# chrischoy/DeepGlobalRegistration

Hardware: AMD Instinct MI355X
Metric: pair registrations/sec (FCGF x2 + 1-NN + 6-D inlier net + gate + weighted Procrustes + SE(3) refinement) (higher is better)
Workload: dtype f32 results via 2 x f16 split operands (3 f16 MFMA products per MAC, f32 accumulate); k = 1 convs, kNN re-evaluation and registration in exact f32, SVD in f64

## Files before the change

deepglobalregistration_amd/csrc/conv_wide.hip:

```cpp
#include <stdlib.h>

#include <type_traits>

#include "dgr_internal.h"
#include "split.h"

struct ConvWideArgs {
  const unsigned char *planes;
  const float *row_scale;
  float *y;
  const uint4 *wb;
  int64_t piece_stride;
  const int32_t *pair_in, *tile_ptr;
  int cout, K;
  float w_unscale;
  unsigned long long *clk;
};

#define DGR_LDS_PTR(off) ((__attribute__((address_space(3))) void *)(lds + (off)))
#define DGR_GLOBAL_PTR(p) ((const __attribute__((address_space(1))) void *)(p))

template <int N>
__device__ __forceinline__ void dgr_wait_vmcnt() {
  static_assert(N >= 0 && N < 64, "vmcnt is a 6-bit counter");
  asm volatile("s_waitcnt vmcnt(%0)" ::"n"(N) : "memory");
}
__device__ __forceinline__ void dgr_phase_barrier() {
  asm volatile("s_waitcnt lgkmcnt(0)\n\ts_barrier" ::: "memory");
}

__host__ __device__ constexpr int dgr_wide_passes(int h, int npass, int nsp) {
  return h < nsp ? npass / nsp + (h < npass % nsp ? 1 : 0) : 0;
}
__host__ __device__ constexpr int dgr_wide_pass_base(int h, int npass, int nsp) {
  int b = 0;
  for (int i = 0; i < h; ++i) b += dgr_wide_passes(i, npass, nsp);
  return b;
}

template <int CP, int NB, int WM>
__global__ void __launch_bounds__(512, 1) sparse_conv_wide_f16x2(ConvWideArgs a, const int4 *__restrict__ tdesc) {
  constexpr int NCW = 4;
  constexpr int NP = 2, MB = 2 / WM, WN = NCW / WM, PW = 4, TM = 64, CK = 64, SK = CK / 16;
  static_assert(WM == 1 || WM == 2, "row split of the compute waves");
  static_assert(TM == DGR_TILE_M && CP % CK == 0, "shape");
  constexpr int PPT = CP / CK, S = CP / 16, NBLK = NB * WN, COUT = 32 * NBLK;
  static_assert(PPT == 1 || PPT == 2 || PPT == 4, "a round of NSET phases is a whole number of tiles");
  constexpr int ROWB = 4 * CP;
  constexpr int NBUF = 3;
  constexpr int NSET = 4;
  constexpr int LEAD = NSET + 2;
  constexpr int BUFB = TM * 256;
  constexpr int RING = 16;
  constexpr int AH_I = 8, AH_S = 4;
  static_assert(RING >= 2 * AH_I && AH_I > LEAD && AH_S >= 3 && AH_S < AH_I, "ring distances");
  constexpr int WD = NB >= 2 ? 2 : 4;
  static_assert(SK % WD == 0, "the weight ring turns a whole number of times per phase (static register indexing)");
  constexpr int LDS_ST = COUT + 4;
  constexpr int NSTG = PPT == 1 ? 2 : 1;
  constexpr int HB = PPT / 2;
  constexpr int RPH = TM / PPT;
  constexpr int PD = 2;
  constexpr int PTH = 64 * (PW - PD);
  constexpr int CPR = COUT / 4;
  constexpr int RPP = PTH / CPR;
  constexpr int NPS = RPH / RPP;
  static_assert(RPH % RPP == 0, "store passes");
  constexpr int OFF_STAGE = NBUF * BUFB;
  constexpr int OFF_IDX = OFF_STAGE + NSTG * TM * LDS_ST * 4;
  constexpr int OFF_SC = OFF_IDX + RING * TM * 4;
  constexpr int LDS_BYTES = OFF_SC + RING * TM * 4;
  static_assert(LDS_BYTES <= 160 * 1024, "LDS budget");
  __shared__ __attribute__((aligned(16))) unsigned char lds[LDS_BYTES];

  const int tid = threadIdx.x;
  const int lane = tid & 63;
  const int wave = __builtin_amdgcn_readfirstlane(tid >> 6);
  if (a.clk && tid == 0) atomicMin(a.clk, (unsigned long long)wall_clock64());
  const int T = a.tile_ptr[a.K];
  const int per = (T + 7) >> 3;
  const int xcd = blockIdx.x & 7;
  const int t_end = min(T, (xcd + 1) * per);
  const int nj = gridDim.x >> 3;
  const int t_first = xcd * per + (blockIdx.x >> 3);
  if (t_first >= t_end) return;
  const int n_my = (t_end - t_first + nj - 1) / nj;
  const int n_loop = n_my + 2;
  auto desc = [&](int i) -> int4 { return tdesc[t_first + min(max(i, 0), n_my - 1) * nj]; };
  auto stage_of = [&](int t) -> float * {
    return reinterpret_cast<float *>(lds + OFF_STAGE) + (NSTG == 2 ? (t & 1) : 0) * TM * LDS_ST;
  };

  if (wave >= NCW) {
    const int pw = wave - NCW;
    if (pw < PD) {
      constexpr int RW = TM / PD, NI = RW / 4;
      f32x4 G[NSET][NI];
      const unsigned char *rb[NI];
      auto row_bases = [&](int i) {
        const int *idx = reinterpret_cast<const int *>(lds + OFF_IDX + (i & (RING - 1)) * TM * 4);
#pragma unroll
        for (int jj = 0; jj < NI; ++jj) {
          const int r = RW * pw + 4 * jj + (lane >> 4);
          rb[jj] = a.planes + (int64_t)idx[r] * ROWB + 16 * ((lane & 15) ^ (r & 15));
        }
      };
      auto request = [&](int p, f32x4 *Gs) {
        if (p % PPT == 0) row_bases(p / PPT);
#pragma unroll
        for (int jj = 0; jj < NI; ++jj) Gs[jj] = *reinterpret_cast<const f32x4 *>(rb[jj] + (p % PPT) * 256);
      };
      auto land = [&](int p, const f32x4 *Gs) {
        unsigned char *dst = lds + (p % NBUF) * BUFB + (NI * pw) * 1024 + lane * 16;
#pragma unroll
        for (int jj = 0; jj < NI; ++jj) *reinterpret_cast<f32x4 *>(dst + jj * 1024) = Gs[jj];
      };
      int *ring_i = reinterpret_cast<int *>(lds + OFF_IDX);
      float *ring_s = reinterpret_cast<float *>(lds + OFF_SC);
      auto load_idx = [&](int i) -> int {
        const int4 d = desc(i);
        return a.pair_in[d.y + min(lane, d.z - 1)];
      };
#pragma unroll
      for (int i = 0; i < AH_I - 1; ++i) ring_i[i * TM + lane] = load_idx(i);
#pragma unroll
      for (int i = 0; i < AH_S - 1; ++i) ring_s[i * TM + lane] = a.row_scale[ring_i[i * TM + lane]];
      int idx_reg = load_idx(AH_I - 1);
      float sc_reg = a.row_scale[ring_i[(AH_S - 1) * TM + lane]];
      auto rings = [&](int t) {
        ring_i[((t + AH_I - 1) & (RING - 1)) * TM + lane] = idx_reg;
        ring_s[((t + AH_S - 1) & (RING - 1)) * TM + lane] = sc_reg;
        idx_reg = load_idx(t + AH_I);
        sc_reg = a.row_scale[ring_i[((t + AH_S) & (RING - 1)) * TM + lane]];
      };
      dgr_phase_barrier();
#pragma unroll
      for (int j = 0; j < NSET; ++j) request(j, G[j]);
      land(0, G[0]); request(NSET, G[0]);
      land(1, G[1]); request(NSET + 1, G[1]);
      dgr_phase_barrier();
      auto phase = [&](int q, f32x4 *Gs) {
        if (q % PPT == 0) rings(q / PPT);
        land(q + 2, Gs);
        request(q + LEAD, Gs);
        dgr_phase_barrier();
      };
      for (int q = 0; q < n_loop * PPT; q += NSET) {
        phase(q, G[2]);
        if (q + 1 < n_loop * PPT) phase(q + 1, G[3]);
        if (q + 2 < n_loop * PPT) phase(q + 2, G[0]);
        if (q + 3 < n_loop * PPT) phase(q + 3, G[1]);
      }
      return;
    }
    const int ptid = tid - 64 * (NCW + PD);
    auto store_rows = [&](int u, int r0) {
      if (u < 0 || u >= n_my) return;
      const int4 d = desc(u);
      const float *sc = reinterpret_cast<const float *>(lds + OFF_SC + (u & (RING - 1)) * TM * 4);
      const float *st = stage_of(u);
      const int c4 = (ptid % CPR) * 4;
      f32x4 v[NPS];
#pragma unroll
      for (int i = 0; i < NPS; ++i) {
        const int r = r0 + i * RPP + ptid / CPR;
        v[i] = *reinterpret_cast<const f32x4 *>(st + r * LDS_ST + c4);
        v[i] *= dgr_inv_pow2(sc[r]) * a.w_unscale;
      }
#pragma unroll
      for (int i = 0; i < NPS; ++i) {
        const int r = r0 + i * RPP + ptid / CPR;
        if (r < d.z) __builtin_nontemporal_store(v[i], reinterpret_cast<f32x4 *>(a.y + (int64_t)(d.y + r) * COUT + c4));
      }
    };
    dgr_phase_barrier();
    dgr_phase_barrier();
    auto sphase = [&](int t, auto hc) {
      constexpr int h = decltype(hc)::value;
      if constexpr (h == 0) store_rows(t - 2, (PPT - 1) * RPH);
      else store_rows(t - 1, (h - 1) * RPH);
      dgr_phase_barrier();
    };
    for (int t = 0; t < n_loop; ++t) {
      sphase(t, std::integral_constant<int, 0>());
      if constexpr (PPT > 1) sphase(t, std::integral_constant<int, 1>());
      if constexpr (PPT > 2) {
        sphase(t, std::integral_constant<int, 2>());
        sphase(t, std::integral_constant<int, 3>());
      }
    }
    if (a.clk && lane == 0) {
      dgr_wait_vmcnt<0>();
      atomicMax(a.clk + 1, (unsigned long long)wall_clock64());
    }
    return;
  }

  const int wn = wave % WN, wm = wave / WN;
  int4 dc = desc(0), dn = desc(1);
  uint4 w[WD][NB][NP];
  auto wload = [&](int k, int s, uint4 (*ws)[NP]) {
    const uint4 *p = a.wb + ((int64_t)(k * S + s) * NBLK + wn * NB) * 64 + lane;
#pragma unroll
    for (int j = 0; j < NB; ++j)
#pragma unroll
      for (int pc = 0; pc < NP; ++pc) ws[j][pc] = p[(int64_t)pc * a.piece_stride + j * 64];
  };
#pragma unroll
  for (int g = 0; g < WD - 1; ++g) wload(dc.x, g % S, w[g]);
  dgr_phase_barrier();
  dgr_phase_barrier();
  uint4 op[2][MB][NP];
  const int lofs0 = (32 * MB * wm + (lane & 31)) * 256 + 16 * ((lane >> 5) ^ (lane & 15));
  auto oload = [&](int b, int s, uint4 (*o)[NP]) {
    const unsigned char *p = lds + b * BUFB + (lofs0 ^ (32 * s));
    const unsigned char *pm = lds + b * BUFB + (lofs0 ^ (32 * s) ^ 128);
#pragma unroll
    for (int i = 0; i < MB; ++i) {
      o[i][0] = *reinterpret_cast<const uint4 *>(p + i * 32 * 256);
      o[i][1] = *reinterpret_cast<const uint4 *>(pm + i * 32 * 256);
    }
  };
  oload(0, 0, op[0]);
  int buf = 0;
  constexpr int NPC = (4 * NB + SK - 1) / SK;
  auto stage_pieces = [&](float *st, const f32x16 (&ac)[MB][NB], int i, int s) {
    float *dst = st + (32 * (MB * wm + i) + (lane & 31)) * LDS_ST;
#pragma unroll
    for (int u = 0; u < NPC; ++u) {
      const int wq = s * NPC + u, j = wq / 4, g = wq % 4;
      if (wq < 4 * NB) {
        const int col = 32 * (wn * NB + j) + 8 * g + 4 * (lane >> 5);
        *reinterpret_cast<f32x4 *>(dst + col) = f32x4{ac[i][j][4 * g], ac[i][j][4 * g + 1], ac[i][j][4 * g + 2], ac[i][j][4 * g + 3]};
      }
    }
  };
  auto ctile = [&](int t, f32x16 (&ac)[MB][NB], const f32x16 (&ad)[MB][NB]) {
    const bool stage_prev = t >= 1 && t <= n_my;
    float *st = stage_of(t - 1);
#pragma unroll
    for (int h = 0; h < PPT; ++h) {
      if (h == 0) {
#pragma unroll
        for (int i = 0; i < MB; ++i)
#pragma unroll
          for (int j = 0; j < NB; ++j)
#pragma unroll
            for (int e = 0; e < 16; ++e) ac[i][j][e] = 0.f;
      }
      const int nbuf = buf == NBUF - 1 ? 0 : buf + 1;
      const int s0 = h * SK;
#pragma unroll
      for (int s = 0; s < SK; ++s) {
        {
          const int sg = s0 + s + WD - 1;
          wload(sg < S ? dc.x : dn.x, sg < S ? sg : sg - S, w[(s + WD - 1) % WD]);
        }
        if (s + 1 < SK) oload(buf, s + 1, op[(s + 1) & 1]);
        else oload(nbuf, 0, op[0]);
        __builtin_amdgcn_sched_barrier(0);
        uint4 (*wc)[NP] = w[s % WD];
        uint4 (*oc)[NP] = op[s & 1];
#define DGR_WIDE_TERM(WP, OP)                                                                                         \
  _Pragma("unroll") for (int i = 0; i < MB; ++i) _Pragma("unroll") for (int j = 0; j < NB; ++j)                       \
      ac[i][j] = __builtin_amdgcn_mfma_f32_32x32x16_f16(__builtin_bit_cast(f16x8, wc[j][WP]),                          \
                                                        __builtin_bit_cast(f16x8, oc[i][OP]), ac[i][j], 0, 0, 0);
        DGR_WIDE_TERM(1, 0)
        DGR_WIDE_TERM(0, 1)
        DGR_WIDE_TERM(0, 0)
#undef DGR_WIDE_TERM
        if (stage_prev) {
          if (h == 0) stage_pieces(st, ad, 0, s);
          if constexpr (MB > 1) {
            if (h == HB) stage_pieces(st, ad, 1, s);
          }
        }
      }
      if (h == PPT - 1) {
        dc = dn;
        dn = desc(t + 2);
      }
      buf = nbuf;
      dgr_phase_barrier();
    }
  };
  f32x16 accA[MB][NB], accB[MB][NB];
  for (int t = 0; t < n_loop; t += 2) {
    ctile(t, accA, accB);
    if (t + 1 < n_loop) ctile(t + 1, accB, accA);
  }
  if (a.clk && lane == 0) atomicMax(a.clk + 1, (unsigned long long)wall_clock64());
}

template <int CP, int NB, int WM>
static int launch_wide(const ConvWideArgs &ka, const int4 *tile_desc, int64_t tile_bound, int num_cus, hipStream_t stream) {
  int64_t grid = num_cus;
  if (tile_bound < grid) grid = tile_bound;
  grid = (grid + 7) / 8 * 8;
  if (grid < 8) grid = 8;
  sparse_conv_wide_f16x2<CP, NB, WM><<<(int)grid, 512, 0, stream>>>(ka, tile_desc);
  DGR_LAUNCH_CHECK();
  return DGR_OK;
}

bool dgr_conv_wide_supported(int cin_pad, int cin, int cout) {
  if (cin != cin_pad) return false;
  return (cout == 64 && cin == 64) || (cout == 128 && (cin == 64 || cin == 128 || cin == 256)) ||
         (cout == 256 && (cin == 128 || cin == 256));
}

int dgr_conv_wide_launch(const DgrConvLaunch &a, const DgrSplitRows &in, const void *wb, int64_t piece_stride,
                         float w_unscale, int num_cus, hipStream_t stream, const char **kernel_name) {
  DGR_REQUIRE(a.pair_in && wb && in.planes && in.scale && dgr_conv_wide_supported(a.cin_pad, a.cin, a.cout),
              "wide conv: unsupported layer (Cin %d, Cout %d) or no split input rows", a.cin, a.cout);
  DGR_REQUIRE(in.channels == a.cin, "wide conv: the split rows have %d channels, the layer %d", in.channels, a.cin);
  DGR_REQUIRE(a.y, "wide conv: no product-row buffer");
  ConvWideArgs ka;
  ka.planes = in.planes; ka.row_scale = in.scale; ka.y = a.y;
  ka.wb = static_cast<const uint4 *>(wb); ka.piece_stride = piece_stride;
  ka.pair_in = a.pair_in; ka.tile_ptr = a.tile_ptr; ka.cout = a.cout; ka.K = a.K; ka.w_unscale = w_unscale;
  ka.clk = a.clk;
  const int64_t tile_bound = a.tile_bound > 0 ? a.tile_bound : (int64_t)num_cus * 4;
#define DGR_WIDE(CPV, NBV, WMV)                                                                 \
  do {                                                                                          \
    if (kernel_name) *kernel_name = "sparse_conv_wide_f16x2<" #CPV ", " #NBV ", " #WMV ">";     \
    return launch_wide<CPV, NBV, WMV>(ka, a.tile_desc, tile_bound, num_cus, stream);            \
  } while (0)
  if (a.cout == 64 && a.cin == 64) DGR_WIDE(64, 1, 2);
  if (a.cout == 128 && a.cin == 64) DGR_WIDE(64, 1, 1);
  if (a.cout == 128 && a.cin == 128) DGR_WIDE(128, 1, 1);
  if (a.cout == 128 && a.cin == 256) DGR_WIDE(256, 1, 1);
  if (a.cout == 256 && a.cin == 128) DGR_WIDE(128, 2, 1);
  if (a.cout == 256 && a.cin == 256) DGR_WIDE(256, 2, 1);
#undef DGR_WIDE
  dgr_set_error("wide conv: no kernel for Cin %d, Cout %d", a.cin, a.cout);
  return DGR_EINVAL;
}

template <int LPR, bool SPLIT>
__global__ void __launch_bounds__(256) row_scale_kernel(const float *__restrict__ in, int in_ld, int cin, int relu,
                                                        const int32_t *__restrict__ n_dev, float *__restrict__ out,
                                                        unsigned char *__restrict__ planes, uint32_t *__restrict__ amax_out) {
  constexpr int RPW = 64 / LPR;
  const int lane = threadIdx.x & 63;
  const int sub = lane / LPR, l = lane % LPR;
  const int n = *n_dev;
  const int relu_lo = relu ? 0 : (int)0x80000000;
  const int64_t stride = (int64_t)gridDim.x * 4 * RPW;
  for (int64_t r0 = ((int64_t)blockIdx.x * 4 + (threadIdx.x >> 6)) * RPW; r0 < n; r0 += stride) {
    const int64_t r = r0 + sub;
    uint32_t mx = 0;
    if (r < n) {
      const float *row = in + r * in_ld;
      for (int c = l * 4; c < cin; c += LPR * 4) {
        mx = max(mx, dgr_abs_max4(__builtin_bit_cast(i32x4, *reinterpret_cast<const f32x4 *>(row + c)), relu_lo));
      }
    }
    mx = dgr_lane_max<LPR>(mx);
    const float sx = dgr_row_scale_of(mx);
    if (l == 0 && r < n) {
      if (out) out[r] = sx;
      if (amax_out) amax_out[r] = mx;
    }
    if constexpr (SPLIT) {
      if (r < n) {
        const float *row = in + r * in_ld;
        unsigned char *dst = planes + r * 4 * cin;
        for (int c = l * 4; c < cin; c += LPR * 4) {
          const i32x4 v = __builtin_bit_cast(i32x4, *reinterpret_cast<const f32x4 *>(row + c));
          f16x4 h, m;
#pragma unroll
          for (int u = 0; u < 4; ++u) {
            _Float16 hh, mm;
            dgr_split2(__builtin_bit_cast(float, max(v[u], relu_lo)), sx, hh, mm);
            h[u] = hh; m[u] = mm;
          }
          *reinterpret_cast<f16x4 *>(dst + dgr_split_row_offset(c, 0)) = h;
          *reinterpret_cast<f16x4 *>(dst + dgr_split_row_offset(c, 1)) = m;
        }
      }
    }
  }
}

static int row_scale_launch(const float *in, int in_ld, int cin, int relu, const int32_t *n_dev, int64_t n_cap, float *out,
                            unsigned char *planes, uint32_t *amax_out, hipStream_t stream) {
  DGR_REQUIRE((cin & 3) == 0 && (in_ld & 3) == 0 && cin >= 4, "row scale: channel count and row stride must be multiples of 4");
  const int lpr = cin >= 256 ? 64 : cin >= 128 ? 32 : cin >= 64 ? 16 : cin >= 32 ? 8 : 4;
  int64_t grid = dgr_ceil_div(n_cap, 4 * (64 / lpr));
  if (grid > 4096) grid = 4096;
  if (grid < 1) grid = 1;
#define DGR_RS(L)                                                                                                   \
  do {                                                                                                              \
    if (planes) row_scale_kernel<L, true><<<(int)grid, 256, 0, stream>>>(in, in_ld, cin, relu, n_dev, out, planes, amax_out); \
    else row_scale_kernel<L, false><<<(int)grid, 256, 0, stream>>>(in, in_ld, cin, relu, n_dev, out, nullptr, amax_out);      \
  } while (0)
  switch (lpr) {
    case 64: DGR_RS(64); break;
    case 32: DGR_RS(32); break;
    case 16: DGR_RS(16); break;
    case 8: DGR_RS(8); break;
    default: DGR_RS(4); break;
  }
#undef DGR_RS
  DGR_LAUNCH_CHECK();
  return DGR_OK;
}

int dgr_row_amax(const float *in, int in_ld, int cin, int relu, const int32_t *n_dev, int64_t n_cap, uint32_t *out,
                 hipStream_t stream) {
  return row_scale_launch(in, in_ld, cin, relu, n_dev, n_cap, nullptr, nullptr, out, stream);
}

int dgr_split_rows(const float *in, int in_ld, int relu, const int32_t *n_dev, int64_t n_cap, const DgrSplitRows &out,
                   hipStream_t stream) {
  DGR_REQUIRE(out.planes && out.scale && out.channels % 64 == 0, "split rows: need planes, scales and a multiple of 64 channels");
  return row_scale_launch(in, in_ld, out.channels, relu, n_dev, n_cap, out.scale, out.planes, nullptr, stream);
}
```

deepglobalregistration_amd/csrc/net.hip:

```cpp
#include <math.h>
#include <stdlib.h>
#include <string.h>

#include <algorithm>
#include <map>
#include <memory>
#include <string>

#include "dgr_internal.h"

static const int CH[5] = {0, 32, 64, 128, 256};
static const int TR[5] = {0, 64, 64, 64, 128};
static constexpr float BN_EPS = 1e-5f;

struct DgrLayer {
  std::string name;
  int K, cin, cout, cin_pad, cout_pad;
  float *w = nullptr;
  float *w16 = nullptr;
  void *w16b = nullptr;
  void *w16d = nullptr;
  int64_t w16b_piece = 0;
  float *wc = nullptr;
  float *wq = nullptr;
// ... 724 lines not shown
  DGR_CHECK(f.conv(li++, V4, &ms.same[2], false, 2, 2, S4T, &U4));
  DGR_CHECK(f.conv(li++, CAT4, &ms.down[1], true, 2, 1, U2, nullptr));
  DGR_CHECK(f.conv(li++, U2, &ms.same[1], false, 1, 1, V2, nullptr));
  DGR_CHECK(f.conv(li++, V2, &ms.same[1], false, 1, 1, S2T, &U2));
  DGR_CHECK(f.conv(li++, CAT2, &ms.down[0], true, 1, 0, U1, nullptr));
  DGR_CHECK(f.conv(li++, U1, &ms.same[0], false, 0, 0, V1, nullptr));
  DGR_CHECK(f.conv(li++, V1, &ms.same[0], false, 0, 0, S1T, &U1));
  const Tensor CAT1{cat1, 96, 1};
  DGR_CHECK(f.conv(li++, CAT1, nullptr, false, 0, 0, H, nullptr));
  f.l2_next = fuse_l2;
  DGR_CHECK(f.conv(li++, H, nullptr, false, 0, 0, FIN, nullptr));
  if (net->normalize && !fuse_l2)
    DGR_CHECK(dgr_l2_normalize_rows(fin, net->cout, out, net->cout, net->cout, 0, ms.cm[0].n_dev, n1, stream));

  auto &I = net->inter;
  net->run_generation = ctx->arena.generation;
  I.clear();
  I["s1"] = {S1.ptr, 96, 32, ms.cm[0].n_dev};
  I["s2"] = {S2.ptr, 128, 64, ms.cm[1].n_dev, ms.cm[1].canon};
  I["s4"] = {S4.ptr, 256, 128, ms.cm[2].n_dev, ms.cm[2].canon};
  I["s8"] = {S8.ptr, 256, 256, ms.cm[3].n_dev, ms.cm[3].canon};
  I["s4_tr"] = {cat4, 256, 128, ms.cm[2].n_dev, ms.cm[2].canon};
  I["s2_tr"] = {cat2, 128, 64, ms.cm[1].n_dev, ms.cm[1].canon};
  I["s1_tr"] = {cat1, 96, 64, ms.cm[0].n_dev};
  auto reg =[&](const char *name, const Tensor &t, int cols, int lvl) {
    DgrTensorRec r;
    r.f32 = (t.split_only || t.dsplit_only) ? nullptr : t.ptr;
    r.ld = t.ld; r.cols = cols;
    r.amax = t.amax;
    r.planes = t.split.planes; r.scale = t.split.scale;
    r.dsplit = t.dsplit;
    r.n_dev = ms.cm[lvl].n_dev; r.canon = ms.cm[lvl].canon;
    net->tensors[name] = r;
  };
  reg("T1", T1, 32, 0); reg("Y1", Y1, 32, 0); reg("S1", S1, 32, 0);
  reg("T2", T2, 64, 1); reg("Y2", Y2, 64, 1); reg("S2", S2, 64, 1);
  reg("T4", T4, 128, 2); reg("Y4", Y4, 128, 2); reg("S4", S4, 128, 2);
  reg("T8", T8, 256, 3); reg("Y8", Y8, 256, 3); reg("S8", S8, 256, 3);
  reg("U4", U4, 128, 2); reg("V4", V4, 128, 2); reg("S4T", S4T, 128, 2); reg("CAT4", CAT4, 256, 2);
  reg("U2", U2, 64, 1); reg("V2", V2, 64, 1); reg("S2T", S2T, 64, 1); reg("CAT2", CAT2, 128, 1);
  reg("U1", U1, 64, 0); reg("V1", V1, 64, 0); reg("S1T", S1T, 64, 0); reg("CAT1", CAT1, 96, 0);
  reg("H", H, 64, 0);
  reg("OUT", Tensor{out, net->cout, 0}, net->cout, 0);

  return DGR_OK;
}

void dgr_ctx_begin_profile(dgr_ctx *ctx) {
  ctx->events.used = 0;
  ctx->conv_spans.clear();
  ctx->gemm_spans.clear();
  ctx->conv_kinds.clear();
  ctx->conv_clks.clear();
  ctx->map3_spans.clear();
  ctx->map6_spans.clear();
  ctx->conv_launches = 0;
}

int dgr_ctx_collect_profile(dgr_ctx *ctx) {
  auto total = [](const std::vector<std::pair<hipEvent_t, hipEvent_t>> &v, float *out) -> int {
    float s = 0.f, t = 0.f;
    for (auto &sp : v) {
      DGR_HIP_CHECK(hipEventElapsedTime(&t, sp.first, sp.second));
      s += t;
    }
    *out = s;
    return DGR_OK;
  };
  DGR_CHECK(total(ctx->map3_spans, &ctx->stage_ms[5]));
  DGR_CHECK(total(ctx->map6_spans, &ctx->stage_ms[6]));
  DGR_CHECK(total(ctx->conv_spans, &ctx->stage_ms[7]));
  ctx->conv_launches = (int64_t)ctx->conv_spans.size();
  ctx->conv_span_ms.clear();
  ctx->gemm_span_ms.clear();
  for (auto &sp : ctx->conv_spans) {
    float t = 0.f;
    DGR_HIP_CHECK(hipEventElapsedTime(&t, sp.first, sp.second));
    ctx->conv_span_ms.push_back(t);
  }
  for (auto &sp : ctx->gemm_spans) {
    float t = 0.f;
    DGR_HIP_CHECK(hipEventElapsedTime(&t, sp.first, sp.second));
    ctx->gemm_span_ms.push_back(t);
  }
  ctx->conv_clk_us.assign(ctx->conv_spans.size(), 0.f);
  for (size_t i = 0; i < ctx->conv_clks.size() && i < ctx->conv_clk_us.size(); ++i)
    if (ctx->conv_clks[i]) {
      unsigned long long c[2] = {0, 0};
      DGR_HIP_CHECK(hipMemcpy(c, ctx->conv_clks[i], sizeof(c), hipMemcpyDeviceToHost));
      if (c[1] > c[0]) ctx->conv_clk_us[i] = (float)((double)(c[1] - c[0]) * 0.01);
    }
  return DGR_OK;
}

int dgr_flag_error(int32_t flag) {
  if (flag == 1) {
    dgr_set_error("duplicate coordinates in the sparse tensor input");
    return DGR_EINVAL;
  }
  if (flag == 2) {
    dgr_set_error("kernel-map capacity exceeded (more than the reserved pairs per output row)");
    return DGR_ENOMEM;
  }
  return DGR_OK;
}

static int check_flag(dgr_ctx *ctx, const int32_t *flag_dev, hipStream_t stream) {
  unsigned char *pin;
  DGR_CHECK(dgr_ctx_pinned(ctx, 64, &pin));
  DGR_HIP_CHECK(hipMemcpyAsync(pin, flag_dev, sizeof(int32_t), hipMemcpyDeviceToHost, stream));
  DGR_CHECK(dgr_ctx_wait(ctx, stream));
  return dgr_flag_error(*reinterpret_cast<volatile int32_t *>(pin));
}

int dgr_ctx_new_flag(dgr_ctx *ctx, hipStream_t stream) {
  DGR_ALLOC(ctx->flag_dev, ctx->arena, int32_t, 1);
  DGR_HIP_CHECK(hipMemsetAsync(ctx->flag_dev, 0, sizeof(int32_t), stream));
  return DGR_OK;
}

int dgr_ctx_check_flag(dgr_ctx *ctx, hipStream_t stream) {
  if (!ctx->flag_dev) return DGR_OK;
  return check_flag(ctx, ctx->flag_dev, stream);
}

void dgr_net_invalidate_runs(dgr_net *net) { net->run_generation = ~0ull; }
int dgr_net_out_channels(const dgr_net *net) { return net->cout; }
int dgr_net_in_channels(const dgr_net *net) { return net->cin; }
int dgr_net_dim(const dgr_net *net) { return net->D; }
const dgr_ctx *dgr_net_ctx(const dgr_net *net) { return net->ctx; }

extern "C" int dgr_resunet_forward(dgr_ctx *ctx, dgr_net *net, const int32_t *coords, const float *feats,
                                   int64_t N, float *out, dgr_stream stream_) {
  DGR_REQUIRE(ctx && net && coords && feats && out, "dgr_resunet_forward: NULL argument");
  DGR_REQUIRE(net->ctx == ctx, "dgr_resunet_forward: the net object belongs to another context (one dgr_net per context: "
                               "dgr_net_share gives a second context its own over the same weights)");
  DGR_REQUIRE(N > 0, "dgr_resunet_forward: empty sparse tensor (N=%lld)", (long long)N);
  hipStream_t stream = (hipStream_t)stream_;
  DGR_HIP_CHECK(hipSetDevice(ctx->device));
  DGR_CHECK(ctx->arena.reset());
  DGR_CHECK(dgr_ctx_new_flag(ctx, stream));
  dgr_ctx_begin_profile(ctx);
  DGR_CHECK(dgr_resunet_forward_impl(ctx, net, coords, feats, N, out, stream));
  DGR_CHECK(dgr_ctx_check_flag(ctx, stream));
  if (ctx->profiling) {
    memset(ctx->stage_ms, 0, sizeof(ctx->stage_ms));
    DGR_CHECK(dgr_ctx_collect_profile(ctx));
  }
  return DGR_OK;
}

extern "C" int dgr_debug_conv_layer(dgr_ctx *ctx, dgr_net *net, int layer, const int32_t *coords, const float *in,
                                    int in_relu, int64_t N, float *out, dgr_stream stream_) {
  DGR_REQUIRE(ctx && net && coords && in && out && N > 0, "dgr_debug_conv_layer: bad argument");
  DGR_REQUIRE(layer >= 0 && layer < (int)net->W->layers.size(), "layer %d out of range", layer);
  const DgrLayer &L = net->W->layers[layer];
  int k3 = 1;
  for (int d = 0; d < net->D; ++d) k3 *= 3;
  DGR_REQUIRE(L.K == k3 && L.cin >= 32, "dgr_debug_conv_layer: layer %s is not a 3^D conv with >= 32 input channels", L.name.c_str());
  hipStream_t stream = (hipStream_t)stream_;
  DGR_HIP_CHECK(hipSetDevice(ctx->device));
  DGR_CHECK(ctx->arena.reset());
  DGR_CHECK(dgr_ctx_new_flag(ctx, stream));
  dgr_ctx_begin_profile(ctx);
  DgrArena &A = ctx->arena;
  Fwd f;
  f.ctx = ctx; f.net = net; f.stream = stream; f.prof = false;
  f.ms.overflow = ctx->flag_dev;
  DGR_CHECK(dgr_build_maps(A, coords, N, net->D, 3, &f.ms, stream, false, true, net->D == 3));
  const int64_t n_cap = f.ms.cm[0].n_cap;
  if (!f.ms.use_nbr) DGR_ALLOC(f.ybuf, A, float, f.ms.same[0].pair_cap * L.cout);
  Tensor tin{const_cast<float *>(in), L.cin, in_relu}, tout{out, L.cout, 0};
  if (L.wb) {
    tin.split.channels = L.cin;
    DGR_ALLOC(tin.split.planes, A, unsigned char, (size_t)n_cap * 4 * L.cin);
    DGR_ALLOC(tin.split.scale, A, float, n_cap);
    DGR_CHECK(dgr_split_rows(in, L.cin, in_relu, f.ms.cm[0].n_dev, n_cap, tin.split, stream));
  }
  DGR_CHECK(f.conv(layer, tin, &f.ms.same[0], false, 0, 0, tout, nullptr));
  DGR_CHECK(dgr_ctx_check_flag(ctx, stream));
  dgr_net_invalidate_runs(net);
  return DGR_OK;
}

extern "C" int dgr_net_get_intermediate(dgr_ctx *ctx, dgr_net *net, const char *name, float *host_out,
                                        int64_t capacity, int64_t *rows, int64_t *cols) {
  DGR_REQUIRE(ctx && net && name && rows && cols, "NULL argument");
  auto it = net->inter.find(name);
  DGR_REQUIRE(it != net->inter.end() && it->second.n_dev, "no intermediate named '%s' (run a forward first)", name);
  DGR_REQUIRE(net->run_generation == ctx->arena.generation,
              "the activations of the last forward are gone: a later call on this context reused its workspace");
  const DgrTensorRef &t = it->second;
  int32_t n = 0;
  DGR_HIP_CHECK(hipDeviceSynchronize());
  DGR_HIP_CHECK(hipMemcpy(&n, t.n_dev, sizeof(int32_t), hipMemcpyDeviceToHost));
  *rows = n;
  *cols = t.cols;
  if (host_out) {
    DGR_REQUIRE(capacity >= (int64_t)n * t.cols, "host buffer too small");
    if (!t.canon) {
      DGR_HIP_CHECK(hipMemcpy2D(host_out, (size_t)t.cols * sizeof(float), t.ptr, (size_t)t.ld * sizeof(float),
                                (size_t)t.cols * sizeof(float), (size_t)n, hipMemcpyDeviceToHost));
    } else {
      std::vector<float> tmp((size_t)n * t.cols);
      std::vector<int32_t> canon(n);
      DGR_HIP_CHECK(hipMemcpy2D(tmp.data(), (size_t)t.cols * sizeof(float), t.ptr, (size_t)t.ld * sizeof(float),
                                (size_t)t.cols * sizeof(float), (size_t)n, hipMemcpyDeviceToHost));
      DGR_HIP_CHECK(hipMemcpy(canon.data(), t.canon, (size_t)n * sizeof(int32_t), hipMemcpyDeviceToHost));
      for (int32_t p = 0; p < n; ++p)
        memcpy(host_out + (size_t)canon[p] * t.cols, tmp.data() + (size_t)p * t.cols, (size_t)t.cols * sizeof(float));
    }
    for (int64_t i = 0; i < (int64_t)n * t.cols; ++i) host_out[i] = host_out[i] > 0.f ? host_out[i] : 0.f;
  }
  return DGR_OK;
}

extern "C" int dgr_net_get_tensor(dgr_ctx *ctx, dgr_net *net, const char *name, int repr, void *host_out,
                                  int64_t capacity_bytes, int64_t *rows, int64_t *row_bytes) {
  DGR_REQUIRE(ctx && net && name && rows && row_bytes, "NULL argument");
  auto it = net->tensors.find(name);
  DGR_REQUIRE(it != net->tensors.end() && it->second.n_dev, "no tensor named '%s' (run a forward first)", name);
  DGR_REQUIRE(net->run_generation == ctx->arena.generation,
              "the activations of the last forward are gone: a later call on this context reused its workspace");
  const DgrTensorRec &t = it->second;
  const void *src = nullptr;
  size_t rb = 0, ld = 0;
  const char *what = "";
  switch (repr) {
    case DGR_TENSOR_F32: src = t.f32; rb = (size_t)t.cols * 4; ld = (size_t)t.ld * 4; what = "f32 rows"; break;
    case DGR_TENSOR_AMAX: src = t.amax; rb = ld = 4; what = "row maxima"; break;
    case DGR_TENSOR_SPLIT_PLANES: src = t.planes; rb = ld = (size_t)t.cols * 4; what = "split rows"; break;
    case DGR_TENSOR_SPLIT_SCALE: src = t.scale; rb = ld = 4; what = "split-row scales"; break;
    case DGR_TENSOR_DENSE_SPLIT: src = t.dsplit; rb = ld = (size_t)t.cols * 4; what = "dense split rows"; break;
    default: DGR_REQUIRE(false, "dgr_net_get_tensor: unknown representation %d", repr);
  }
  DGR_REQUIRE(src != nullptr, "the last forward did not write tensor '%s' as %s", name, what);
  int32_t n = 0;
  DGR_HIP_CHECK(hipDeviceSynchronize());
  DGR_HIP_CHECK(hipMemcpy(&n, t.n_dev, sizeof(int32_t), hipMemcpyDeviceToHost));
  *rows = n;
  *row_bytes = (int64_t)rb;
  if (!host_out) return DGR_OK;
  DGR_REQUIRE(capacity_bytes >= (int64_t)n * (int64_t)rb, "host buffer too small");
  if (!t.canon) {
    DGR_HIP_CHECK(hipMemcpy2D(host_out, rb, src, ld, rb, (size_t)n, hipMemcpyDeviceToHost));
  } else {
    std::vector<unsigned char> tmp((size_t)n * rb);
    std::vector<int32_t> canon(n);
    DGR_HIP_CHECK(hipMemcpy2D(tmp.data(), rb, src, ld, rb, (size_t)n, hipMemcpyDeviceToHost));
    DGR_HIP_CHECK(hipMemcpy(canon.data(), t.canon, (size_t)n * sizeof(int32_t), hipMemcpyDeviceToHost));
    for (int32_t p = 0; p < n; ++p) {
      DGR_REQUIRE(canon[p] >= 0 && canon[p] < n, "dgr_net_get_tensor: row numbering out of range");
      memcpy(static_cast<unsigned char *>(host_out) + (size_t)canon[p] * rb, tmp.data() + (size_t)p * rb, rb);
    }
  }
  return DGR_OK;
}

extern "C" int dgr_net_layer_stats(dgr_ctx *ctx, dgr_net *net, int layer, int64_t stats[8]) {
  DGR_REQUIRE(ctx && net && stats, "NULL argument");
  DGR_REQUIRE(layer >= 0 && layer < (int)net->W->layers.size(), "layer %d out of range", layer);
  const LayerRun &r = net->runs[layer];
  DGR_REQUIRE(r.n_in && r.n_out, "run a forward first");
  DGR_REQUIRE(net->run_generation == ctx->arena.generation,
              "the kernel maps of the last forward are gone: a later call on this context reused its workspace");
  const DgrLayer &L = net->W->layers[layer];
  DGR_HIP_CHECK(hipDeviceSynchronize());
  int32_t n_in = 0, n_out = 0;
  DGR_HIP_CHECK(hipMemcpy(&n_in, r.n_in, sizeof(int32_t), hipMemcpyDeviceToHost));
  DGR_HIP_CHECK(hipMemcpy(&n_out, r.n_out, sizeof(int32_t), hipMemcpyDeviceToHost));
  int64_t P = n_out, kne = 1;
  if (r.os) {
    int64_t counts[27];
    DGR_CHECK(dgr_nbr_counts(r.nbr, r.n_out, counts));
    P = 0;
    kne = 0;
    for (int k = 0; k < 27; ++k) { P += counts[k]; kne += counts[k] > 0; }
  } else if (r.fused_pairs) {
    int32_t pc = 0;
    DGR_HIP_CHECK(hipMemcpy(&pc, r.fused_pairs, sizeof(int32_t), hipMemcpyDeviceToHost));
    P = pc;
    kne = r.K;
  } else if (r.rule_ptr) {
    std::vector<int32_t> rp(r.K + 1);
    DGR_HIP_CHECK(hipMemcpy(rp.data(), r.rule_ptr, (size_t)(r.K + 1) * sizeof(int32_t), hipMemcpyDeviceToHost));
    P = rp[r.K];
    kne = 0;
    for (int k = 0; k < r.K; ++k) kne += rp[k + 1] > rp[k];
  }
  stats[0] = P; stats[1] = kne; stats[2] = n_in; stats[3] = n_out;
  stats[4] = L.cin; stats[5] = L.cout; stats[6] = L.K; stats[7] = 0;
  return DGR_OK;
}

extern "C" int dgr_net_rerun_layer(dgr_ctx *ctx, dgr_net *net, int layer, int reps, float *gemm_ms, float *reduce_ms) {
  DGR_REQUIRE(ctx && net && gemm_ms && reduce_ms && reps > 0, "bad argument");
  DGR_REQUIRE(layer >= 0 && layer < (int)net->W->layers.size(), "layer %d out of range", layer);
  const LayerRun &r = net->runs[layer];
  DGR_REQUIRE(r.n_in && r.n_out, "run a forward first");
  DGR_REQUIRE(net->run_generation == ctx->arena.generation,
              "the kernel maps of the last forward are gone: a later call on this context reused its workspace");
  DGR_REQUIRE(!r.fused_pairs, "layer %d ran fused with its neighbour search; not re-runnable", layer);
  const DgrLayer &L = net->W->layers[layer];
  hipEvent_t e0, e1, e2;
  DGR_HIP_CHECK(hipEventCreate(&e0)); DGR_HIP_CHECK(hipEventCreate(&e1)); DGR_HIP_CHECK(hipEventCreate(&e2));
  float tg = 0.f, tr = 0.f;
  for (int i = 0; i < reps + 1; ++i) {
    DGR_HIP_CHECK(hipEventRecord(e0, nullptr));
    if (r.os)
      DGR_CHECK(dgr_conv_os_launch(r.os_launch, nullptr));
    else if (r.small_cin)
      DGR_CHECK(dgr_conv_small_cin(r.launch.in, r.launch.in_ld, r.launch.in_relu, L.cin, L.w, L.wq, L.shift, r.km, r.n_out,
                                   r.n_out_cap, r.launch.out, r.launch.out_ld, nullptr));
    else if (L.wb && r.has_reduce)
      DGR_CHECK(dgr_conv_wide_launch(r.launch, r.split_in, L.wb, L.wb_piece, L.w_unscale, ctx->num_cus, nullptr));
    else
      DGR_CHECK(dgr_conv_launch(r.launch, ctx->num_cus, nullptr));
    DGR_HIP_CHECK(hipEventRecord(e1, nullptr));
    if (r.has_reduce && !r.small_cin && !r.os)
      DGR_CHECK(dgr_reduce_rows(r.launch.y, L.cout, r.red_ptr, r.red_pos, r.n_out, r.n_out_cap,
                                r.split_only ? nullptr : r.launch.out, r.launch.out_ld, L.shift, r.res, r.res_ld, r.res_relu, nullptr,
                                r.split_out.planes ? &r.split_out : nullptr, r.out_relu));
    DGR_HIP_CHECK(hipEventRecord(e2, nullptr));
    DGR_HIP_CHECK(hipEventSynchronize(e2));
    float a = 0.f, b = 0.f;
    DGR_HIP_CHECK(hipEventElapsedTime(&a, e0, e1));
    DGR_HIP_CHECK(hipEventElapsedTime(&b, e1, e2));
    if (i > 0) { tg += a; tr += b; }
  }
  (void)hipEventDestroy(e0); (void)hipEventDestroy(e1); (void)hipEventDestroy(e2);
  *gemm_ms = tg / reps;
  *reduce_ms = tr / reps;
  return DGR_OK;
}
```

Measured before the change: 390.2.

## Use a half-step weight ring and split operand loads in the wide sparse conv

For the NB=2 wide conv shapes, weights are now prefetched one column block at a time through an 8-deep register ring instead of whole steps. Part of the next operand's LDS load is deferred into the middle of the MFMA sequence. This is meant to shorten weight-load stalls and lower register pressure in the compute waves. The producer's index and scale ring is generalised, with a deeper 32-entry ring and lookahead derived from NSET and PPT. The change also adds optional compile-time stage clock instrumentation and moves the layer re-run timing helper onto the context's part stream; the added schedule complexity could worsen latency hiding.

```diff
diff --git a/deepglobalregistration_amd/csrc/conv_wide.hip b/deepglobalregistration_amd/csrc/conv_wide.hip
--- a/deepglobalregistration_amd/csrc/conv_wide.hip
+++ b/deepglobalregistration_amd/csrc/conv_wide.hip
@@ -29,6 +29,40 @@
   asm volatile("s_waitcnt lgkmcnt(0)\n\ts_barrier" ::: "memory");
 }
 
+#ifdef DGR_WIDE_STAGE_CLK
+__device__ unsigned long long dgr_wide_stage_clk[6][16];
+extern "C" int dgr_debug_wide_stage_clk(unsigned long long *out96, int reset) {
+  if (out96 && hipMemcpyFromSymbol(out96, HIP_SYMBOL(dgr_wide_stage_clk), 96 * sizeof(unsigned long long)) != hipSuccess) return -1;
+  if (reset) {
+    unsigned long long z[96] = {0};
+    if (hipMemcpyToSymbol(HIP_SYMBOL(dgr_wide_stage_clk), z, sizeof(z)) != hipSuccess) return -1;
+  }
+  return 0;
+}
+#define DGR_WIDE_CLK(...) __VA_ARGS__
+#define DGR_WIDE_NOW() ((unsigned long long)__builtin_amdgcn_s_memtime())
+#else
+#define DGR_WIDE_CLK(...)
+#endif
+__device__ __forceinline__ void dgr_wide_barrier(unsigned long long &waited) {
+#ifdef DGR_WIDE_STAGE_CLK
+  asm volatile("s_waitcnt lgkmcnt(0)" ::: "memory");
+  const unsigned long long t = DGR_WIDE_NOW();
+  dgr_phase_barrier();
+  waited += DGR_WIDE_NOW() - t;
+#else
+  dgr_phase_barrier();
+#endif
+}
+__host__ __device__ constexpr int dgr_wide_shape_id(int cp, int nb, int wm) {
+  return wm == 2 ? 0 : nb == 2 ? (cp == 128 ? 4 : 5) : cp == 64 ? 1 : cp == 128 ? 2 : 3;
+}
+__host__ __device__ constexpr int dgr_wide_lcm(int a, int b) {
+  int m = a;
+  while (m % b) m += a;
+  return m;
+}
+
 __host__ __device__ constexpr int dgr_wide_passes(int h, int npass, int nsp) {
   return h < nsp ? npass / nsp + (h < npass % nsp ? 1 : 0) : 0;
 }
@@ -38,7 +72,7 @@
   return b;
 }
 
-template <int CP, int NB, int WM>
+template <int CP, int NB, int WM, int NSET, int HD>
 __global__ void __launch_bounds__(512, 1) sparse_conv_wide_f16x2(ConvWideArgs a, const int4 *__restrict__ tdesc) {
   constexpr int NCW = 4;
   constexpr int NP = 2, MB = 2 / WM, WN = NCW / WM, PW = 4, TM = 64, CK = 64, SK = CK / 16;
@@ -48,14 +82,15 @@
   static_assert(PPT == 1 || PPT == 2 || PPT == 4, "a round of NSET phases is a whole number of tiles");
   constexpr int ROWB = 4 * CP;
   constexpr int NBUF = 3;
-  constexpr int NSET = 4;
   constexpr int LEAD = NSET + 2;
   constexpr int BUFB = TM * 256;
-  constexpr int RING = 16;
-  constexpr int AH_I = 8, AH_S = 4;
-  static_assert(RING >= 2 * AH_I && AH_I > LEAD && AH_S >= 3 && AH_S < AH_I, "ring distances");
+  constexpr int DI = PPT == 1 ? 1 : (NSET + PPT - 1) / PPT;
+  constexpr int AH_S = DI + 2, AH_I = 2 * DI + 3 > DI + (LEAD + PPT - 1) / PPT ? 2 * DI + 3 : DI + (LEAD + PPT - 1) / PPT;
+  constexpr int RING = 32;
+  static_assert(AH_I - DI > AH_S && (AH_I - DI) * PPT >= LEAD && AH_S - DI >= 2 && RING >= AH_I + 4, "ring distances");
   constexpr int WD = NB >= 2 ? 2 : 4;
-  static_assert(SK % WD == 0, "the weight ring turns a whole number of times per phase (static register indexing)");
+  static_assert(S % WD == 0 && WD - 1 <= S, "the weight ring turns a whole number of times per tile (static register indexing)");
+  static_assert(HD == 0 || (NB == 2 && (2 * S) % HD == 0 && HD >= 2), "half-step weight ring");
   constexpr int LDS_ST = COUT + 4;
   constexpr int NSTG = PPT == 1 ? 2 : 1;
   constexpr int HB = PPT / 2;
@@ -122,35 +157,52 @@
         return a.pair_in[d.y + min(lane, d.z - 1)];
       };
 #pragma unroll
-      for (int i = 0; i < AH_I - 1; ++i) ring_i[i * TM + lane] = load_idx(i);
-#pragma unroll
-      for (int i = 0; i < AH_S - 1; ++i) ring_s[i * TM + lane] = a.row_scale[ring_i[i * TM + lane]];
-      int idx_reg = load_idx(AH_I - 1);
-      float sc_reg = a.row_scale[ring_i[(AH_S - 1) * TM + lane]];
-      auto rings = [&](int t) {
-        ring_i[((t + AH_I - 1) & (RING - 1)) * TM + lane] = idx_reg;
-        ring_s[((t + AH_S - 1) & (RING - 1)) * TM + lane] = sc_reg;
-        idx_reg = load_idx(t + AH_I);
-        sc_reg = a.row_scale[ring_i[((t + AH_S) & (RING - 1)) * TM + lane]];
+      for (int i = 0; i < AH_I - DI; ++i) ring_i[i * TM + lane] = load_idx(i);
+#pragma unroll
+      for (int i = 0; i < AH_S - DI; ++i) ring_s[i * TM + lane] = a.row_scale[ring_i[i * TM + lane]];
+      int idx_reg[DI];
+      float sc_reg[DI];
+#pragma unroll
+      for (int d = 0; d < DI; ++d) idx_reg[d] = load_idx(AH_I - DI + d);
+#pragma unroll
+      for (int d = 0; d < DI; ++d) sc_reg[d] = a.row_scale[ring_i[(AH_S - DI + d) * TM + lane]];
+      auto rings = [&](int t, int &ir, float &sr) {
+        ring_i[((t + AH_I - DI) & (RING - 1)) * TM + lane] = ir;
+        ring_s[((t + AH_S - DI) & (RING - 1)) * TM + lane] = sr;
+        ir = load_idx(t + AH_I);
+        sr = a.row_scale[ring_i[((t + AH_S) & (RING - 1)) * TM + lane]];
       };
+      DGR_WIDE_CLK(const unsigned long long life0 = DGR_WIDE_NOW(); unsigned long long c_land = 0, c_rings = 0;)
+      unsigned long long c_bar = 0;
       dgr_phase_barrier();
 #pragma unroll
       for (int j = 0; j < NSET; ++j) request(j, G[j]);
       land(0, G[0]); request(NSET, G[0]);
       land(1, G[1]); request(NSET + 1, G[1]);
       dgr_phase_barrier();
-      auto phase = [&](int q, f32x4 *Gs) {
-        if (q % PPT == 0) rings(q / PPT);
+      auto phase = [&](int q, bool first, f32x4 *Gs, int &ir, float &sr) {
+        DGR_WIDE_CLK(const unsigned long long t0 = DGR_WIDE_NOW();)
+        if (first) rings(q / PPT, ir, sr);
+        DGR_WIDE_CLK(const unsigned long long t1 = DGR_WIDE_NOW();)
         land(q + 2, Gs);
+        DGR_WIDE_CLK(c_rings += t1 - t0; c_land += DGR_WIDE_NOW() - t1;)
         request(q + LEAD, Gs);
-        dgr_phase_barrier();
+        dgr_wide_barrier(c_bar);
       };
-      for (int q = 0; q < n_loop * PPT; q += NSET) {
-        phase(q, G[2]);
-        if (q + 1 < n_loop * PPT) phase(q + 1, G[3]);
-        if (q + 2 < n_loop * PPT) phase(q + 2, G[0]);
-        if (q + 3 < n_loop * PPT) phase(q + 3, G[1]);
-      }
+      constexpr int ROUND = dgr_wide_lcm(NSET, PPT * DI);
+      for (int q = 0; q < n_loop * PPT; q += ROUND) {
+#pragma unroll
+        for (int j = 0; j < ROUND; ++j) {
+          if (q + j < n_loop * PPT) phase(q + j, j % PPT == 0, G[(j + 2) % NSET], idx_reg[(j / PPT) % DI], sc_reg[(j / PPT) % DI]);
+        }
+      }
+#ifdef DGR_WIDE_STAGE_CLK
+      if (lane == 0) {
+        unsigned long long *c = dgr_wide_stage_clk[dgr_wide_shape_id(CP, NB, WM)];
+        atomicAdd(c + 4, c_bar); atomicAdd(c + 5, c_land); atomicAdd(c + 6, c_rings);
+        atomicAdd(c + 7, DGR_WIDE_NOW() - life0); atomicAdd(c + 8, 1ull);
+      }
+#endif
       return;
     }
     const int ptid = tid - 64 * (NCW + PD);
@@ -173,13 +225,15 @@
         if (r < d.z) __builtin_nontemporal_store(v[i], reinterpret_cast<f32x4 *>(a.y + (int64_t)(d.y + r) * COUT + c4));
       }
     };
+    DGR_WIDE_CLK(const unsigned long long life0 = DGR_WIDE_NOW();)
+    unsigned long long c_bar = 0;
     dgr_phase_barrier();
     dgr_phase_barrier();
     auto sphase = [&](int t, auto hc) {
       constexpr int h = decltype(hc)::value;
       if constexpr (h == 0) store_rows(t - 2, (PPT - 1) * RPH);
       else store_rows(t - 1, (h - 1) * RPH);
-      dgr_phase_barrier();
+      dgr_wide_barrier(c_bar);
     };
     for (int t = 0; t < n_loop; ++t) {
       sphase(t, std::integral_constant<int, 0>());
@@ -193,34 +247,52 @@
       dgr_wait_vmcnt<0>();
       atomicMax(a.clk + 1, (unsigned long long)wall_clock64());
     }
+#ifdef DGR_WIDE_STAGE_CLK
+    if (lane == 0) {
+      unsigned long long *c = dgr_wide_stage_clk[dgr_wide_shape_id(CP, NB, WM)];
+      atomicAdd(c + 9, c_bar); atomicAdd(c + 10, DGR_WIDE_NOW() - life0); atomicAdd(c + 11, 1ull);
+    }
+#endif
     return;
   }
 
   const int wn = wave % WN, wm = wave / WN;
   int4 dc = desc(0), dn = desc(1);
-  uint4 w[WD][NB][NP];
+  constexpr int NW = HD > 0 ? HD : WD * NB;
+  uint4 w[NW][NP];
+  auto wload1 = [&](int k, int s, int j, uint4 *ws) {
+    const uint4 *p = a.wb + ((int64_t)(k * S + s) * NBLK + wn * NB + j) * 64 + lane;
+#pragma unroll
+    for (int pc = 0; pc < NP; ++pc) ws[pc] = p[(int64_t)pc * a.piece_stride];
+  };
   auto wload = [&](int k, int s, uint4 (*ws)[NP]) {
-    const uint4 *p = a.wb + ((int64_t)(k * S + s) * NBLK + wn * NB) * 64 + lane;
-#pragma unroll
-    for (int j = 0; j < NB; ++j)
-#pragma unroll
-      for (int pc = 0; pc < NP; ++pc) ws[j][pc] = p[(int64_t)pc * a.piece_stride + j * 64];
+#pragma unroll
+    for (int j = 0; j < NB; ++j) wload1(k, s, j, ws[j]);
   };
-#pragma unroll
-  for (int g = 0; g < WD - 1; ++g) wload(dc.x, g % S, w[g]);
+  if constexpr (HD > 0) {
+#pragma unroll
+    for (int g = 0; g < HD - 1; ++g) wload1(dc.x, (g / 2) % S, g % 2, w[g]);
+  } else {
+#pragma unroll
+    for (int g = 0; g < WD - 1; ++g) wload(dc.x, g % S, &w[g * NB]);
+  }
+  DGR_WIDE_CLK(const unsigned long long life0 = DGR_WIDE_NOW(), wall0 = wall_clock64(); unsigned long long c_w = 0;)
+  unsigned long long c_bar = 0;
   dgr_phase_barrier();
   dgr_phase_barrier();
   uint4 op[2][MB][NP];
   const int lofs0 = (32 * MB * wm + (lane & 31)) * 256 + 16 * ((lane >> 5) ^ (lane & 15));
-  auto oload = [&](int b, int s, uint4 (*o)[NP]) {
+  constexpr bool XM1 = HD >= 8;
+  auto oload_part = [&](int b, int s, uint4 (*o)[NP], bool xh, bool xm) {
     const unsigned char *p = lds + b * BUFB + (lofs0 ^ (32 * s));
     const unsigned char *pm = lds + b * BUFB + (lofs0 ^ (32 * s) ^ 128);
 #pragma unroll
     for (int i = 0; i < MB; ++i) {
-      o[i][0] = *reinterpret_cast<const uint4 *>(p + i * 32 * 256);
-      o[i][1] = *reinterpret_cast<const uint4 *>(pm + i * 32 * 256);
+      if (xh) o[i][0] = *reinterpret_cast<const uint4 *>(p + i * 32 * 256);
+      if (xm) o[i][1] = *reinterpret_cast<const uint4 *>(pm + i * 32 * 256);
     }
   };
+  auto oload = [&](int b, int s, uint4 (*o)[NP]) { oload_part(b, s, o, true, true); };
   oload(0, 0, op[0]);
   int buf = 0;
   constexpr int NPC = (4 * NB + SK - 1) / SK;
@@ -252,23 +324,59 @@
       const int s0 = h * SK;
 #pragma unroll
       for (int s = 0; s < SK; ++s) {
-        {
-          const int sg = s0 + s + WD - 1;
-          wload(sg < S ? dc.x : dn.x, sg < S ? sg : sg - S, w[(s + WD - 1) % WD]);
+        uint4 (*oc)[NP] = op[s & 1];
+#define DGR_WIDE_WEIGHT_WAIT(W0, W1)                                                                                  \
+  DGR_WIDE_CLK(__builtin_amdgcn_sched_barrier(0);                                                                     \
+               asm volatile("" ::"v"(__builtin_bit_cast(f16x8, (W0)[0])), "v"(__builtin_bit_cast(f16x8, (W0)[1])),     \
+                            "v"(__builtin_bit_cast(f16x8, (W1)[0])), "v"(__builtin_bit_cast(f16x8, (W1)[1])));         \
+               const unsigned long long tw1 = DGR_WIDE_NOW(); __builtin_amdgcn_sched_barrier(0);)
+#define DGR_WIDE_TERM(WP, OX, J0, J1, WJ)                                                                             \
+  _Pragma("unroll") for (int i = 0; i < MB; ++i) _Pragma("unroll") for (int j = J0; j < J1; ++j)                      \
+      ac[i][j] = __builtin_amdgcn_mfma_f32_32x32x16_f16(__builtin_bit_cast(f16x8, (WJ)[WP]),                           \
+                                                        __builtin_bit_cast(f16x8, OX), ac[i][j], 0, 0, 0);
+        if constexpr (HD == 0) {
+          {
+            const int sg = s0 + s + WD - 1;
+            wload(sg < S ? dc.x : dn.x, sg < S ? sg : sg - S, &w[(sg % WD) * NB]);
+          }
+          DGR_WIDE_CLK(const unsigned long long tw0 = DGR_WIDE_NOW();)
+          if (s + 1 < SK) oload(buf, s + 1, op[(s + 1) & 1]);
+          else oload(nbuf, 0, op[0]);
+          __builtin_amdgcn_sched_barrier(0);
+          uint4 (*wc)[NP] = &w[((s0 + s) % WD) * NB];
+          DGR_WIDE_WEIGHT_WAIT(wc[0], wc[NB - 1])
+          DGR_WIDE_TERM(1, oc[i][0], 0, NB, wc[j])
+          DGR_WIDE_TERM(0, oc[i][1], 0, NB, wc[j])
+          DGR_WIDE_TERM(0, oc[i][0], 0, NB, wc[j])
+          DGR_WIDE_CLK(__builtin_amdgcn_sched_barrier(0); c_w += tw1 - tw0;)
+        } else {
+#pragma unroll
+          for (int jb = 0; jb < 2; ++jb) {
+            constexpr int G2 = 2 * S;
+            const int g = 2 * (s0 + s) + jb, gg = g + HD - 1;
+            wload1(gg < G2 ? dc.x : dn.x, (gg % G2) / 2, gg % 2, w[gg % HD]);
+            DGR_WIDE_CLK(const unsigned long long tw0 = DGR_WIDE_NOW();)
+            if (jb == 0) {
+              if (s + 1 < SK) oload_part(buf, s + 1, op[(s + 1) & 1], true, !XM1);
+              else oload_part(nbuf, 0, op[0], true, !XM1);
+            }
+            __builtin_amdgcn_sched_barrier(0);
+            uint4 *wc = w[g % HD];
+            DGR_WIDE_WEIGHT_WAIT(wc, wc)
+            DGR_WIDE_TERM(1, oc[i][0], jb, jb + 1, wc)
+            DGR_WIDE_TERM(0, op[XM1 ? 0 : s & 1][i][1], jb, jb + 1, wc)
+            if (XM1 && jb == 1) {
+              __builtin_amdgcn_sched_barrier(0);
+              if (s + 1 < SK) oload_part(buf, s + 1, op[0], false, true);
+              else oload_part(nbuf, 0, op[0], false, true);
+              __builtin_amdgcn_sched_barrier(0);
+            }
+            DGR_WIDE_TERM(0, oc[i][0], jb, jb + 1, wc)
+            DGR_WIDE_CLK(__builtin_amdgcn_sched_barrier(0); c_w += tw1 - tw0;)
+          }
         }
-        if (s + 1 < SK) oload(buf, s + 1, op[(s + 1) & 1]);
-        else oload(nbuf, 0, op[0]);
-        __builtin_amdgcn_sched_barrier(0);
-        uint4 (*wc)[NP] = w[s % WD];
-        uint4 (*oc)[NP] = op[s & 1];
-#define DGR_WIDE_TERM(WP, OP)                                                                                         \
-  _Pragma("unroll") for (int i = 0; i < MB; ++i) _Pragma("unroll") for (int j = 0; j < NB; ++j)                       \
-      ac[i][j] = __builtin_amdgcn_mfma_f32_32x32x16_f16(__builtin_bit_cast(f16x8, wc[j][WP]),                          \
-                                                        __builtin_bit_cast(f16x8, oc[i][OP]), ac[i][j], 0, 0, 0);
-        DGR_WIDE_TERM(1, 0)
-        DGR_WIDE_TERM(0, 1)
-        DGR_WIDE_TERM(0, 0)
 #undef DGR_WIDE_TERM
+#undef DGR_WIDE_WEIGHT_WAIT
         if (stage_prev) {
           if (h == 0) stage_pieces(st, ad, 0, s);
           if constexpr (MB > 1) {
@@ -281,7 +389,7 @@
         dn = desc(t + 2);
       }
       buf = nbuf;
-      dgr_phase_barrier();
+      dgr_wide_barrier(c_bar);
     }
   };
   f32x16 accA[MB][NB], accB[MB][NB];
@@ -290,15 +398,26 @@
     if (t + 1 < n_loop) ctile(t + 1, accB, accA);
   }
   if (a.clk && lane == 0) atomicMax(a.clk + 1, (unsigned long long)wall_clock64());
-}
-
-template <int CP, int NB, int WM>
+#ifdef DGR_WIDE_STAGE_CLK
+  if (lane == 0) {
+    unsigned long long *c = dgr_wide_stage_clk[dgr_wide_shape_id(CP, NB, WM)];
+    const unsigned long long life = DGR_WIDE_NOW() - life0;
+    atomicAdd(c + 0, c_bar); atomicAdd(c + 1, c_w); atomicAdd(c + 2, life); atomicAdd(c + 3, 1ull);
+    if (wave == 0) {
+      atomicAdd(c + 12, (unsigned long long)(n_loop * PPT)); atomicAdd(c + 13, life);
+      atomicAdd(c + 14, (unsigned long long)wall_clock64() - wall0);
+    }
+  }
+#endif
+}
+
+template <int CP, int NB, int WM, int NSET, int HD>
 static int launch_wide(const ConvWideArgs &ka, const int4 *tile_desc, int64_t tile_bound, int num_cus, hipStream_t stream) {
   int64_t grid = num_cus;
   if (tile_bound < grid) grid = tile_bound;
   grid = (grid + 7) / 8 * 8;
   if (grid < 8) grid = 8;
-  sparse_conv_wide_f16x2<CP, NB, WM><<<(int)grid, 512, 0, stream>>>(ka, tile_desc);
+  sparse_conv_wide_f16x2<CP, NB, WM, NSET, HD><<<(int)grid, 512, 0, stream>>>(ka, tile_desc);
   DGR_LAUNCH_CHECK();
   return DGR_OK;
 }
@@ -324,7 +443,7 @@
 #define DGR_WIDE(CPV, NBV, WMV)                                                                 \
   do {                                                                                          \
     if (kernel_name) *kernel_name = "sparse_conv_wide_f16x2<" #CPV ", " #NBV ", " #WMV ">";     \
-    return launch_wide<CPV, NBV, WMV>(ka, a.tile_desc, tile_bound, num_cus, stream);            \
+    return launch_wide<CPV, NBV, WMV, 4, (NBV == 2 ? 8 : 0)>(ka, a.tile_desc, tile_bound, num_cus, stream); \
   } while (0)
   if (a.cout == 64 && a.cin == 64) DGR_WIDE(64, 1, 2);
   if (a.cout == 128 && a.cin == 64) DGR_WIDE(64, 1, 1);
diff --git a/deepglobalregistration_amd/csrc/net.hip b/deepglobalregistration_amd/csrc/net.hip
--- a/deepglobalregistration_amd/csrc/net.hip
+++ b/deepglobalregistration_amd/csrc/net.hip
@@ -1050,26 +1050,27 @@
               "the kernel maps of the last forward are gone: a later call on this context reused its workspace");
   DGR_REQUIRE(!r.fused_pairs, "layer %d ran fused with its neighbour search; not re-runnable", layer);
   const DgrLayer &L = net->W->layers[layer];
+  hipStream_t st = ctx->part_stream;
   hipEvent_t e0, e1, e2;
   DGR_HIP_CHECK(hipEventCreate(&e0)); DGR_HIP_CHECK(hipEventCreate(&e1)); DGR_HIP_CHECK(hipEventCreate(&e2));
   float tg = 0.f, tr = 0.f;
   for (int i = 0; i < reps + 1; ++i) {
-    DGR_HIP_CHECK(hipEventRecord(e0, nullptr));
+    DGR_HIP_CHECK(hipEventRecord(e0, st));
     if (r.os)
-      DGR_CHECK(dgr_conv_os_launch(r.os_launch, nullptr));
+      DGR_CHECK(dgr_conv_os_launch(r.os_launch, st));
     else if (r.small_cin)
       DGR_CHECK(dgr_conv_small_cin(r.launch.in, r.launch.in_ld, r.launch.in_relu, L.cin, L.w, L.wq, L.shift, r.km, r.n_out,
-                                   r.n_out_cap, r.launch.out, r.launch.out_ld, nullptr));
+                                   r.n_out_cap, r.launch.out, r.launch.out_ld, st));
     else if (L.wb && r.has_reduce)
-      DGR_CHECK(dgr_conv_wide_launch(r.launch, r.split_in, L.wb, L.wb_piece, L.w_unscale, ctx->num_cus, nullptr));
+      DGR_CHECK(dgr_conv_wide_launch(r.launch, r.split_in, L.wb, L.wb_piece, L.w_unscale, ctx->num_cus, st));
     else
-      DGR_CHECK(dgr_conv_launch(r.launch, ctx->num_cus, nullptr));
-    DGR_HIP_CHECK(hipEventRecord(e1, nullptr));
+      DGR_CHECK(dgr_conv_launch(r.launch, ctx->num_cus, st));
+    DGR_HIP_CHECK(hipEventRecord(e1, st));
     if (r.has_reduce && !r.small_cin && !r.os)
       DGR_CHECK(dgr_reduce_rows(r.launch.y, L.cout, r.red_ptr, r.red_pos, r.n_out, r.n_out_cap,
-                                r.split_only ? nullptr : r.launch.out, r.launch.out_ld, L.shift, r.res, r.res_ld, r.res_relu, nullptr,
+                                r.split_only ? nullptr : r.launch.out, r.launch.out_ld, L.shift, r.res, r.res_ld, r.res_relu, st,
                                 r.split_out.planes ? &r.split_out : nullptr, r.out_relu));
-    DGR_HIP_CHECK(hipEventRecord(e2, nullptr));
+    DGR_HIP_CHECK(hipEventRecord(e2, st));
     DGR_HIP_CHECK(hipEventSynchronize(e2));
     float a = 0.f, b = 0.f;
     DGR_HIP_CHECK(hipEventElapsedTime(&a, e0, e1));
```

New measurement: 401.2 (median of 6 runs). 2.8% higher.
